# instadeepai/FrameDiPT

Hardware: AMD Instinct MI355X
Metric: residue*diffusion-steps/sec (higher is better)
Workload: dtype fp16

## Files before the change

### framedipt_amd/_lib.py

```python
from __future__ import annotations

import ctypes as C
import os

_HERE = os.path.dirname(os.path.abspath(__file__))
LIB_PATH = os.environ.get("FDIPT_LIB") or os.path.join(_HERE, "lib", "libfdipt_hip.so")

PREC_F32, PREC_BF16, PREC_F16 = 0, 1, 2
PREC_F16X = 3
KF_ET3, KF_GENERIC_PAIR, KF_GENERIC_ATTN, KF_UNFUSED_NODE, KF_UNFOLDED, KF_NO_SPLIT, KF_NO_MERGE, KF_ROWS32, KF_PASS_Z = 1, 2, 4, 8, 16, 32, 64, 128, 256
KF_POINTS_LAUNCH = 512
KF_STREAM_ATTN = 1024
_ERR = {-1: "FDIPT_EINVAL (bad argument)", -2: "FDIPT_ELAUNCH (HIP launch error)",
        -3: "FDIPT_ESIZE (workspace too small or N beyond the compiled tiling: N <= 1024, N <= 2048 with KF_STREAM_ATTN in the fp16 mode; "
            "sample selection: a group of more than 64 samples)"}


class FdiptError(RuntimeError):
    pass


class Dims(C.Structure):
    _fields_ = [(n, C.c_int32) for n in (
        "c_s", "c_z", "c_hidden", "c_skip", "no_heads", "no_qk_points", "no_v_points", "tfmr_heads", "tfmr_layers",
        "num_blocks", "index_embed", "num_bins", "use_aatype", "precision", "kernel_flags")] + [
        (n, C.c_float) for n in ("min_bin", "max_bin", "coordinate_scaling", "r3_min_b", "r3_max_b")]

# ... 153 lines not shown
```

### framedipt_amd/csrc/kernels.hpp

```cpp
#pragma once
#include <hip/hip_runtime.h>
#include <stdint.h>

typedef unsigned short half_t;

struct EdgeTransArgs {
  int B, N;
  const void* z_in;
  void* z_out;
  const float* e;
  const void *w1, *w2, *wf;
  const float *b1, *b2, *bf, *gamma, *beta;
  const float* res_mask;
  float* trace;
  unsigned long long* clock = nullptr;
};

struct EdgeEmbedArgs {
  int B, N, n_rel, rel_off, num_bins;
  const float* pi;
  const float* pj;
  const float* rtab;
  const float* dtab;
  const float* edges;
// ... 212 lines not shown
  float* out = nullptr;
  int ld_out = 0;
  float* out2 = nullptr;
  int ld_out2 = 0, split = 0;
  unsigned short* hid_h16 = nullptr;
  void *img_a = nullptr, *img_b = nullptr;
  int img_B = 0, img_N = 0;
  const float *bb_w = nullptr, *bb_b = nullptr;
  const float* upd_mask = nullptr;
  float *quat = nullptr, *trans = nullptr;
  L2Warm warm = {};
  const void *w3 = nullptr, *w3l = nullptr;
  const float* b3 = nullptr;
  const void *we0 = nullptr, *we0l = nullptr, *we1 = nullptr, *we1l = nullptr;
  const float *be0 = nullptr, *be1 = nullptr;
};
enum { FD_RB_TRANSITION, FD_RB_NODE_EMBED_72, FD_RB_NODE_EMBED_88, FD_RB_TORSION, FD_RB_TRANSITION_BB, FD_RB_ET_ROWS, FD_RB_ET4_ROWS, FD_RB_ET4_IMAGES,
       FD_RB_TRANSITION_BB_SPLIT, FD_RB_NODE_EMBED_72_SPLIT, FD_RB_NODE_EMBED_88_SPLIT, FD_RB_TORSION_SPLIT };
int fd_rowblock(int kind, const RowBlockArgs& a, hipStream_t st);
int fd_transition16(const RowBlockArgs& a, hipStream_t st);
int fd_node_embed16(const RowBlockArgs& a, int k0, hipStream_t st);
int fd_torsion16(const RowBlockArgs& a, hipStream_t st);

struct TfmrTailArgs {
  int M, ld;
  const float *att, *x;
  const void *wo, *w1, *w2;
  const void *wol = nullptr, *w1l = nullptr, *w2l = nullptr, *wpl = nullptr;
  const float *bo, *g1, *be1, *b1, *b2, *g2, *be2;
  float* out;
  const void* wp = nullptr;
  const float *bp = nullptr, *pres = nullptr;
  float* pout = nullptr;
  int ld_pres = 0, ld_pout = 0;
  L2Warm warm;
  int rows16 = 0;
};
int fd_tfmr_tail(const TfmrTailArgs& a, hipStream_t st);
int fd_chain_build_image16(const float* w, int N, int K, int Kpad, int ldw, int lo, void* img, hipStream_t st);

struct ChainArgs {
  int M = 0;
  const float* in = nullptr;
  int ld_in = 0;
  const void* w[3] = {};
  const float* b[3] = {};
  const float* residual = nullptr;
  int ld_res = 0;
  const float *gamma = nullptr, *beta = nullptr;
  unsigned short* out_h16 = nullptr;
  const float* rowmask_pre = nullptr;
  const float* rowmask_post = nullptr;
  float* out = nullptr;
// ... 68 lines not shown
```

### framedipt_amd/csrc/model.hip

```cpp
#include <math.h>
#include <string.h>

#include <vector>

#include "common.hpp"
#include "kernels.hpp"

struct LinW { long w, b; int out, in; };
struct LNW { long g, b; int d; };
#define FD_MAX_BLOCKS 8
#define FD_MAX_TL 4
struct TfLayer { LinW inp, outp, l1, l2; LNW n1, n2; };
struct BlockW {
  long head_w;
  LinW q, kv, qp, kvp, lb, dz, out, rbf;
  LNW ipa_ln;
  LinW skip;
  TfLayer tf[FD_MAX_TL];
  LinW post, t1, t2, t3;
  LNW tln;
  LinW bb;
  LinW et_init, et1, et2, etf;
  LNW et_ln;
};
// ... 565 lines not shown
enum EtRows { ETR_IMAGES, ETR_ROWS, ETR_FOLDED };
struct ForwardPlan {
  int op;
  bool bf, chain, rbk, split;
  NodeForm embed, tail, transition, torsion;
  SkipAt skip;
  OutProj outproj;
  int slices;
  bool feats_fused, ee_bias, et_bias, pz;
  bool stream;
  bool a3, probs_h16;
  bool vpt, proj2, merged, proj_pts, vt_lo, init_fused, feats_h16;
  NodeRows node_rows;
  SeqAttn seq;
  PostAt post;
  bool et_widths;
  EtKind et;
  EtRows et_rows;
  bool torf_fused, bb_fold;
  bool regpair;
  bool ipa_bias_f32, ipa_attn_f32;
  bool x;
  bool refused;
};
static const char kImage = 0;

static ForwardPlan plan_forward(const FdiptDims* d, const Inventory& iv, const DLayout& L, int B, int N, int op) {
  const unsigned f = (unsigned)d->kernel_flags;
  const bool generic_attn = f & FDIPT_KF_GENERIC_ATTN, unfolded = f & FDIPT_KF_UNFOLDED;
  const int cs = d->c_s, cz = d->c_z, H = d->no_heads, C = d->c_hidden, Pq = d->no_qk_points, Pv = d->no_v_points;
// ... 48 lines not shown
  const int th = d->tfmr_heads, hd = iv.d_t / th;
  const bool seq_ok = p.stream ? fd_seq_attention_stream_supported(N, th, hd) : fd_seq_attention_supported(N, th, hd);
  if (p.rbk && !generic_attn && seq_ok && fd_seq_qkv_supported(N, th, iv.d_t)) p.seq = SEQ_FUSED;
  else if (p.bf && !generic_attn && seq_ok) p.seq = SEQ_BF16;
  else if (!p.bf && !generic_attn && fd_seq_attention_f32_supported(N, th, hd, 3 * iv.d_t)) p.seq = SEQ_F32;
  else p.seq = SEQ_GENERIC;
  p.ipa_bias_f32 = !p.bf && H == 8 && cz == 128;
  p.ipa_attn_f32 = !p.bf && !generic_attn;
  p.init_fused = p.proj2 && p.seq == SEQ_FUSED && !unfolded;
  p.feats_h16 = p.a3 && opair_mfma && splitk && (iv.feat_dim & 7) == 0 && !p.split && op == OP_ALL;
  if (!splitk) p.outproj = OUT_GEMM;
  else if (p.split && p.merged && outproj_image(d, iv)) p.outproj = OUT_DEDICATED;
  else p.outproj = p.split ? OUT_SPLITK_SPLIT : p.feats_h16 ? OUT_SPLITK_A16 : OUT_SPLITK;
  p.slices = p.outproj == OUT_DEDICATED ? fd_outproj_split_slices() : p.split ? 3 : 4;
  p.post = p.rbk && !unfolded ? POST_TAIL : p.chain ? POST_CHAIN : POST_GEMM;
  p.torf_fused = (cs & 3) == 0 && !unfolded;
  p.bb_fold = !unfolded;
  p.x = d->precision == FDIPT_PREC_F16X;
  const unsigned x_refused = FDIPT_KF_ET3 | FDIPT_KF_GENERIC_PAIR | FDIPT_KF_GENERIC_ATTN | FDIPT_KF_UNFUSED_NODE | FDIPT_KF_NO_SPLIT |
                             FDIPT_KF_STREAM_ATTN;
  const bool runs_et = op == OP_ALL || op == OP_ET;
  p.refused = p.x && ((f & x_refused) || (runs_et && p.et != ET_ET4) || !p.split || N > 1024);
  return p;
}

enum WarmOf { WARM_QKV, WARM_TAIL, WARM_POST, WARM_TRANSITION, WARM_TRANSITION32, WARM_ET_ROWS, WARM_ET_FOLDED, WARM_TORSION };
struct Fwd {
  const FdiptDims* d;
  const Inventory& iv;
  const DLayout& L;
// ... 17 lines not shown
  int lin32(const LinW& l, const float* A, int lda, float* out, int ldo) const {
    return fd_linear(FDIPT_PREC_F32, R, l.out, l.in, A, lda, P + l.w, l.in, P + l.b, nullptr, 0, nullptr, 0, out, ldo, st);
  }
  int d2d(void* dst, const void* src, size_t bytes) const {
    return hipMemcpyAsync(dst, src, bytes, hipMemcpyDeviceToDevice, st) == hipSuccess ? FDIPT_OK : FDIPT_ELAUNCH;
  }
  int inner(int b, int slot, const float* src, int ld, int cols) const {
    if (!a->trace_inner) return FDIPT_OK;
    float* dst = a->trace_inner + ((size_t)(b * 4 + slot) * R) * iv.d_t;
    return hipMemcpy2DAsync(dst, (size_t)iv.d_t * 4, src, (size_t)ld * 4, (size_t)cols * 4, R, hipMemcpyDeviceToDevice, st) == hipSuccess
               ? FDIPT_OK : FDIPT_ELAUNCH;
  }
  bool first_block(int b) const { return b == 0 || p.op != OP_ALL; }
  bool bias_ready(int b) const { return p.op == OP_ALL && (b == 0 ? p.ee_bias : (p.et == ET_ET3 || p.et == ET_ET4) && p.et_bias); }
  bool fold_et_rows(int b) const { return p.et_rows == ETR_FOLDED && b < d->num_blocks - 1; }
  L2Warm warm_of(int b, WarmOf next, int l = 0) const {
    const DBlock& db = L.blk[b];
    const int cs = d->c_s, dt = iv.d_t;
    const unsigned tb = (unsigned)fd_chain_image_bytes(cs, cs);
    switch (next) {
      case WARM_QKV: {
        const unsigned n = (unsigned)fd_chain_image_bytes(3 * dt, dt);
        return L2Warm{{D + db.ch.inp[l], p.split ? D + db.lo.inp[l] : nullptr, nullptr}, {n, p.split ? n : 0u, 0}};
      }
      case WARM_TAIL: {
        if (p.tail == NF_ROWS16) return L2Warm{{D + db.lo.o16[l][0], D + db.lo.o16[l][1], nullptr}, {db.lo.tail16_run[l], db.lo.tail16_run[l], 0}};
        const unsigned wimg = (unsigned)fd_chain_image_bytes(dt, dt);
        return L2Warm{{D + db.ch.outp[l], D + db.ch.l1[l], D + db.ch.l2[l]}, {wimg, wimg, wimg}};
      }
      case WARM_POST: return L2Warm{{D + db.ch.post, nullptr, nullptr}, {(unsigned)fd_chain_image_bytes(cs, dt), 0, 0}};
// ... 184 lines not shown
    else if (p.outproj == OUT_SPLITK_SPLIT)
      RC(fd_linear_splitk_split(R, cs, feat, p.slices, F(w.feats), feat, wout, feat, bout, res_mask, F(w.ipa_parts), (long)R * cs, cs, st));
    else if (p.outproj == OUT_SPLITK_A16)
      RC(fd_linear_splitk_a16(R, cs, feat, p.slices, (const half_t*)(W + w.feats), feat, WM(k.out), feat, P + k.out.b, res_mask,
                              F(w.ipa_parts), (long)R * cs, cs, st));
    else
      RC(fd_linear_splitk(R, cs, feat, p.slices, F(w.feats), feat, WM(k.out), feat, P + k.out.b, res_mask, F(w.ipa_parts), (long)R * cs, cs, st));
    const bool skip_batched = p.skip != SKIP_PER_BLOCK;
    const L2Warm warm = warm_of(b, WARM_QKV, 0);
    RC(fd_layernorm_parts(R, cs, node, cs, F(w.ipa_parts), cs, p.slices, (long)R * cs, P + k.ipa_ln.g, P + k.ipa_ln.b, nullptr,
                          F(w.tf_in), dt, skip_batched ? F(w.skip_all) + (size_t)b * d->c_skip : nullptr,
                          d->num_blocks * d->c_skip, d->c_skip, p.seq == SEQ_FUSED ? &warm : nullptr, st));
    if (!skip_batched) RC(lin(k.skip, F(w.node0), cs, nullptr, 0, nullptr, 0, F(w.tf_in) + cs, dt));
    return FDIPT_OK;
  }
  int seq_stage(int b, const float** x_out) const {
    const BlockW& k = iv.blk[b];
    const DBlock& db = L.blk[b];
    const int dt = iv.d_t, cs = d->c_s, th = d->tfmr_heads, hd = dt / th;
    const float* x = F(w.tf_in);
    for (int l = 0; l < d->tfmr_layers; ++l) {
      const TfLayer& t = k.tf[l];
      const bool last = l + 1 == d->tfmr_layers;
      if (p.seq == SEQ_FUSED) {
        if (b == 0 && l == 0 && !p.init_fused) RC(fd_seq_images_init(B, N, th, res_mask, W + w.seqimg, SeqInitExtra{}, st, p.stream));
        RC(fd_seq_qkv(B, N, th, x, dt, D + db.ch.inp[l], p.split ? D + db.lo.inp[l] : nullptr, P + t.inp.b, 1.0f / sqrtf((float)hd),
                      W + w.seqimg, st));
        const L2Warm wt = warm_of(b, WARM_TAIL, l);
        RC(fd_seq_attention_run(B, N, th, W + w.seqimg, F(w.att), dt, &wt, st, p.stream));
      } else {
        RC(lin(t.inp, x, dt, nullptr, 0, nullptr, 0, F(w.qkv), 3 * dt));
// ... 18 lines not shown
      const bool r16 = p.tail == NF_ROWS16;
      TfmrTailArgs tt;
      tt.M = R; tt.ld = dt; tt.att = F(w.att); tt.x = x;
      tt.wo = D + (r16 ? db.lo.o16[l][0] : db.ch.outp[l]); tt.w1 = D + (r16 ? db.lo.f16[l][0] : db.ch.l1[l]); tt.w2 = D + (r16 ? db.lo.g16[l][0] : db.ch.l2[l]);
      if (p.split) { tt.wol = D + (r16 ? db.lo.o16[l][1] : db.lo.outp[l]); tt.w1l = D + (r16 ? db.lo.f16[l][1] : db.lo.l1[l]); tt.w2l = D + (r16 ? db.lo.g16[l][1] : db.lo.l2[l]); }
      tt.bo = P + t.outp.b; tt.g1 = P + t.n1.g; tt.be1 = P + t.n1.b; tt.b1 = P + t.l1.b; tt.b2 = P + t.l2.b; tt.g2 = P + t.n2.g;
      tt.be2 = P + t.n2.b; tt.out = x == F(w.x_b) ? F(w.x_a) : F(w.x_b);
      tt.rows16 = r16;
      const bool post_here = last && p.post == POST_TAIL;
      if (post_here) {
        tt.wp = D + (r16 ? db.lo.p16[0] : db.ch.post); tt.wpl = r16 ? D + db.lo.p16[1] : p.split ? D + db.lo.post : nullptr;
        tt.bp = P + k.post.b; tt.pres = F(w.tf_in); tt.ld_pres = dt; tt.pout = F(w.h_a); tt.ld_pout = cs;
      }
      if (!last) tt.warm = p.seq == SEQ_FUSED ? warm_of(b, WARM_QKV, l + 1) : L2Warm{};
      else tt.warm = warm_of(b, post_here ? WARM_TRANSITION : WARM_POST);
      RC(fd_tfmr_tail(tt, st));
      x = tt.out;
    }
    *x_out = x;
    return FDIPT_OK;
  }
  int transition_stage(int b, const float* x) const {
    const BlockW& k = iv.blk[b];
    const DBlock& db = L.blk[b];
    const int cs = d->c_s, dt = iv.d_t;
    if (p.post == POST_CHAIN) {
      ChainArgs c;
      c.M = R; c.in = x; c.ld_in = dt; c.w[0] = D + db.ch.post; c.b[0] = P + k.post.b; c.residual = F(w.tf_in); c.ld_res = dt;
      c.out = F(w.h_a); c.ld_out = cs;
      if (p.rbk) c.warm = warm_of(b, WARM_TRANSITION32);
      RC(fd_chain(FD_CHAIN_POST, c, st));
    } else if (p.post == POST_GEMM) RC(lin(k.post, x, dt, F(w.tf_in), dt, nullptr, 0, F(w.h_a), cs));
    if (p.transition == NF_GEMM) {
      RC(lin(k.t1, F(w.h_a), cs, nullptr, 0, nullptr, 1, F(w.h_b), cs));
      RC(lin(k.t2, F(w.h_b), cs, nullptr, 0, nullptr, 1, F(w.ipa_out), cs));
      RC(lin(k.t3, F(w.ipa_out), cs, F(w.h_a), cs, nullptr, 0, F(w.h_b), cs));
      RC(fd_layernorm(R, cs, F(w.h_b), cs, nullptr, 0, P + k.tln.g, P + k.tln.b, a->res_mask, F(w.node), cs, st));
      RC(lin32(k.bb, F(w.node), cs, F(w.upd), 8));
      RC(inner(b, 3, F(w.upd), 8, 6));
      return fd_compose_q_update(R, F(w.quat), F(w.trans), F(w.upd), 8, F(w.dmask), st);
    }
    const bool r16 = p.transition == NF_ROWS16;
    RowBlockArgs r;
    r.M = R; r.in = F(w.h_a); r.ld_in = cs;
    r.w0 = D + (r16 ? db.lo.tr16[0][0] : db.ch.t1); r.w1 = D + (r16 ? db.lo.tr16[1][0] : db.ch.t2); r.w2 = D + (r16 ? db.lo.tr16[2][0] : db.ch.t3);
    if (p.split) { r.w0l = D + (r16 ? db.lo.tr16[0][1] : db.lo.t1); r.w1l = D + (r16 ? db.lo.tr16[1][1] : db.lo.t2); r.w2l = D + (r16 ? db.lo.tr16[2][1] : db.lo.t3); }
    r.b0 = P + k.t1.b; r.b1 = P + k.t2.b; r.b2 = P + k.t3.b; r.residual = F(w.h_a); r.ld_res = cs; r.gamma = P + k.tln.g; r.beta = P + k.tln.b;
    r.rowmask_post = a->res_mask; r.out = F(w.node); r.ld_out = cs; r.bb_w = P + k.bb.w; r.bb_b = P + k.bb.b;
    r.upd_mask = F(w.dmask); r.quat = F(w.quat); r.trans = F(w.trans);
    if (b < d->num_blocks - 1 && p.et_widths) r.warm = warm_of(b, WARM_ET_ROWS);
    else if (b == d->num_blocks - 1) r.warm = warm_of(b, WARM_TORSION);
    if (fold_et_rows(b)) {
      r.we0 = D + db.lo.ei16[0]; r.we0l = D + db.lo.ei16[1]; r.we1 = D + db.lo.r416[0]; r.we1l = D + db.lo.r416[1];
      r.be0 = P + k.et_init.b; r.be1 = (const float*)(D + db.ch.r4b);
      r.img_a = W + w.a1img; r.img_b = W + w.b1img; r.img_B = B; r.img_N = N;
      r.warm = warm_of(b, WARM_ET_FOLDED);
    }
    if (r16) return fd_transition16(r, st);
    return fd_rowblock(p.split ? FD_RB_TRANSITION_BB_SPLIT : FD_RB_TRANSITION_BB, r, st);
  }
  int edge_transition_stage(int b, const float* node) const {
    const BlockW& k = iv.blk[b];
    const DBlock& db = L.blk[b];
    const int cs = d->c_s, cz = d->c_z;
    RowBlockArgs r;
    r.M = R; r.in = node; r.ld_in = cs; r.w0 = D + db.ch.et_init; r.b0 = P + k.et_init.b;
    if (p.et == ET_ET4 && !fold_et_rows(b)) {
      r.w1 = D + db.ch.r4w; r.b1 = (const float*)(D + db.ch.r4b); r.out = F(w.r4); r.ld_out = 1024;
      r.img_a = W + w.a1img; r.img_b = W + w.b1img; r.img_B = B; r.img_N = N;
      if (p.et_rows == ETR_ROWS) {
        RC(fd_rowblock(FD_RB_ET4_ROWS, r, st));
// ... 34 lines not shown
      t2.clock = a->clock_out;
      if (p.et == ET_ET4) RC(fd_edge_transition4(t2, st, p.x));
      else RC(fd_edge_transition3(t2, st));
    } else {
      EdgeTransArgs ta;
      ta.B = B; ta.N = N; ta.z_in = W + w.z; ta.z_out = W + w.z; ta.e = F(w.e);
      ta.w1 = WM(k.et1); ta.w2 = WM(k.et2); ta.wf = WM(k.etf); ta.b1 = P + k.et1.b; ta.b2 = P + k.et2.b; ta.bf = P + k.etf.b;
      ta.gamma = P + k.et_ln.g; ta.beta = P + k.et_ln.b; ta.res_mask = a->res_mask; ta.trace = tr_ptr; ta.clock = a->clock_out;
      RC(fd_edge_transition(op_precision(d), cz, iv.cb, ta, st));
    }
    if (a->ev_stop && a->ev_stop[b]) hipEventRecord((hipEvent_t)a->ev_stop[b], st);
    return FDIPT_OK;
  }
  int heads_stage(const float* node) const {
    const int cs = d->c_s;
    if (p.torsion == NF_GEMM) {
      RC(lin(iv.tor1, node, cs, nullptr, 0, nullptr, 1, F(w.h_a), cs));
      RC(lin(iv.tor2, F(w.h_a), cs, node, cs, nullptr, 0, F(w.h_b), cs));
    } else {
      const bool r16 = p.torsion == NF_ROWS16;
      RowBlockArgs r;
      r.M = R; r.in = node; r.ld_in = cs; r.w0 = D + (r16 ? L.tor16[0][0] : L.ch_tor1); r.w1 = D + (r16 ? L.tor16[1][0] : L.ch_tor2);
      if (p.split) { r.w0l = D + (r16 ? L.tor16[0][1] : L.lo_tor1); r.w1l = D + (r16 ? L.tor16[1][1] : L.lo_tor2); }
      r.b0 = P + iv.tor1.b; r.b1 = P + iv.tor2.b; r.residual = node; r.ld_res = cs; r.out = F(w.h_b); r.ld_out = cs;
      if (r16) RC(fd_torsion16(r, st));
      else RC(fd_rowblock(p.split ? FD_RB_TORSION_SPLIT : FD_RB_TORSION, r, st));
    }
    if (!p.torf_fused) RC(lin32(iv.torf, F(w.h_b), cs, F(w.psi_un), 8));
    const bool atoms = a->atom37 || a->atom14;
    if (atoms && !a->bb_tables) return FDIPT_EINVAL;
    const bool bb_fold = atoms && p.bb_fold;
// ... 76 lines not shown
    RC(f.ipa_attend(b));
    RC(f.lin(iv.blk[b].out, f.F(w.feats), iv.feat_dim, nullptr, 0, a->res_mask, 0, f.F(w.ipa_out), d->c_s));
    if (!op.out) return FDIPT_EINVAL;
    return f.d2d(op.out, f.F(w.ipa_out), node_bytes);
  }
  const int cs = d->c_s, nsk = d->num_blocks * d->c_skip;
  if (p.skip == SKIP_SPLITK)
    RC(fd_linear_splitk_split(R, nsk, cs, 1, f.F(w.node0), cs, (const float*)(f.D + L.skip_w32), cs, (const float*)(f.D + L.skip_b),
                              nullptr, f.F(w.skip_all), 0, nsk, f.st));
  else if (p.skip == SKIP_GEMM)
    RC(fd_linear(op_precision(d), R, nsk, cs, f.F(w.node0), cs, f.D + L.skip_w, cs, (const float*)(f.D + L.skip_b), nullptr, 0,
                 nullptr, 0, f.F(w.skip_all), nsk, f.st));
  const float* node = f.F(w.node0);
  for (int b = 0; b < d->num_blocks; ++b) {
    const float* x;
    RC(f.ipa_project(b, node));
    RC(f.ipa_attend(b));
    RC(f.ipa_out(b, node));
    RC(f.seq_stage(b, &x));
    RC(f.inner(b, 2, x, iv.d_t, iv.d_t));
    RC(f.transition_stage(b, x));
    node = f.F(w.node);
    if (b < d->num_blocks - 1) RC(f.edge_transition_stage(b, node));
    if (a->trace_node) RC(f.d2d(a->trace_node + (size_t)(b + 1) * R * cs, node, node_bytes));
  }
  return f.heads_stage(node);
}

extern "C" {

int fdipt_score_forward(const FdiptDims* d, const float* P, const void* derived, const void* setup,
                        const FdiptForwardArgs* a, void* workspace, size_t workspace_bytes, fdipt_stream_t stream) {
  return forward_impl(d, P, derived, setup, a, workspace, workspace_bytes, stream, OpSel{});
}

int fdipt_edge_embed_fwd(const FdiptDims* d, const float* P, const void* derived, const void* setup, const FdiptForwardArgs* a,
// ... 56 lines not shown
```

### framedipt_amd/csrc/rowblock.hip

```cpp
#include <type_traits>

#include "common.hpp"
#include "kernels.hpp"

#pragma clang fp contract(off)

#define RB_SROW 144

__host__ __device__ constexpr int rb_max(int a, int b) { return a > b ? a : b; }

template <int K0, int N1, int N2, int NOUT, int FLAGS>
struct RBShape {
  static constexpr int KS0 = (K0 + 15) / 16;
  static constexpr int NL = 1 + (N1 > 0) + (N2 > 0);
  static constexpr int KSMAX = rb_max(KS0, rb_max(N1 / 16, N2 / 16));
  static constexpr int WMAX = rb_max(KS0 * 16, rb_max(N1, N2));
  static constexpr int XROW = WMAX * 2 + 16;
  static constexpr bool LN = (FLAGS & 4) != 0;
  static constexpr int CP = (FLAGS & 64) ? 2 : 1;
  static constexpr int NTO_BLK = NOUT / 32 / CP;
  static constexpr int NTMAX = rb_max(NTO_BLK, rb_max(N1 / 32, N2 / 32));
  static constexpr int NTW = (NTMAX + 3) / 4;
  static constexpr bool BB = (FLAGS & 8) != 0;
  static constexpr bool IMG = (FLAGS & 16) != 0;
// ... 680 lines not shown
        const int r = 8 * it + (lane >> 3);
        const f32x4 o = *(const f32x4*)(stg + r * RB_SROW + 16 * (lane & 7));
        if (row0 + r < a.M) *(f32x4*)(a.out + (long)(row0 + r) * a.ld + 32 * T + 4 * (lane & 7)) = o;
      }
    }
  }
  fd_l2_warm_done(warm_tok);
}

#define RB16_BLOCKS 1
#define T16_KS (TL_D / 32)
#define T16_NT (TL_D / 16)
#define T16_XROW (TL_D * 2 + 32)
#define T16_XLO (16 * T16_XROW)
#define T16_SMEM (4 * T16_XLO + (7 * TL_D + TL_NP) * 4 + 2 * 4 * 16 * 4 + 16)
template <bool POST>
__global__ __launch_bounds__(FD_THREADS, RB16_BLOCKS) void tfmr_tail16_kernel(TfmrTailArgs a) {
  extern __shared__ __attribute__((aligned(16))) char smem[];
  char* xs = smem;
  char* hs = xs + 2 * T16_XLO;
  float* cst = (float*)(hs + 2 * T16_XLO);
  float (*red)[4][16] = (float (*)[4][16])(cst + 7 * TL_D + TL_NP);
  const int tid = threadIdx.x, lane = tid & 63, wave = tid >> 6, lr = lane & 15, fg = lane >> 4;
  const int row0 = blockIdx.x * 16;
  const long grow = row0 + lr < a.M ? row0 + lr : a.M - 1;
  FD_STAMP(0);
  hx8 Wh[2][T16_KS], Wl[2][T16_KS];
  auto w_load = [&](auto BUF, const void* img, const void* img_lo, int T) {
    constexpr int b = decltype(BUF)::value;
#pragma unroll
    for (int s = 0; s < T16_KS; ++s) {
      Wh[b][s] = fd_frag((const char*)img + ((size_t)(T * T16_KS + s) * 64 + lane) * 16);
      Wl[b][s] = fd_frag((const char*)img_lo + ((size_t)(T * T16_KS + s) * 64 + lane) * 16);
// ... 22 lines not shown
      xv[k] = *(const f32x4*)(a.att + (long)gr * a.ld + 4 * c4);
    }
    {
      constexpr int NC = 7 * TL_D + (POST ? TL_NP : 0), NCV = (NC + FD_THREADS - 1) / FD_THREADS;
      float cv[NCV];
#pragma unroll
      for (int k = 0; k < NCV; ++k) {
        const int v = tid + k * FD_THREADS, which = v / TL_D, c = v % TL_D;
        const float* src = which == 0 ? a.bo : which == 1 ? a.g1 : which == 2 ? a.be1 : which == 3 ? a.b1 : which == 4 ? a.b2 : which == 5 ? a.g2 : a.be2;
        cv[k] = v < 7 * TL_D ? src[c] : (POST && v < NC ? a.bp[v - 7 * TL_D] : 0.f);
      }
#pragma unroll
      for (int k = 0; k < NCV; ++k)
        if (tid + k * FD_THREADS < NC) cst[tid + k * FD_THREADS] = cv[k];
    }
#pragma unroll
    for (int k = 0; k < 5; ++k) {
      const int idx = tid + k * FD_THREADS, r = idx / 80, c4 = idx % 80;
      put4(xs, r * T16_XROW + 8 * c4, xv[k][0], xv[k][1], xv[k][2], xv[k][3]);
    }
  }
  f32x4 rv[5];
#pragma unroll
  for (int u = 0; u < 5; ++u) rv[u] = *(const f32x4*)(a.x + grow * a.ld + 16 * (wave + 4 * u) + 4 * fg);
  const unsigned warm_tok = fd_l2_warm(a.warm, blockIdx.x, gridDim.x, tid, FD_THREADS);
  __syncthreads();
  FD_STAMP(1);
  hx8 X[T16_KS];
  const char* xl_base = nullptr;
  auto x_load = [&](const char* buf) {
// ... 113 lines not shown
#pragma unroll
    for (int u = 0; u < 5; ++u)
      put4(hs, lr * T16_XROW + 2 * (16 * (wave + 4 * u) + 4 * fg), acc[u][0], acc[u][1], acc[u][2], acc[u][3]);
    __syncthreads();
    x_load(hs);
#pragma unroll
    for (int u = 0; u < 4; ++u) rvp[u] = *(const f32x4*)(a.pres + grow * a.ld_pres + 16 * (wave + 4 * u) + 4 * fg);
    layer(a.wp, a.wpl, std::integral_constant<int, TL_NP / 16>{});
#pragma unroll
    for (int u = 0; u < 4; ++u) {
      const int f0 = 16 * (wave + 4 * u) + 4 * fg;
      const f32x4 bv = *(const f32x4*)(cst + 7 * TL_D + f0);
      f32x4 o;
#pragma unroll
      for (int i = 0; i < 4; ++i) o[i] = acc[u][i] + bv[i] + rvp[u][i];
      if (row0 + lr < a.M) *(f32x4*)(a.pout + (long)(row0 + lr) * a.ld_pout + f0) = o;
    }
    fd_l2_warm_done(warm_tok);
    return;
  }
#pragma unroll
  for (int u = 0; u < 5; ++u)
    if (row0 + lr < a.M) *(f32x4*)(a.out + (long)(row0 + lr) * a.ld + 16 * (wave + 4 * u) + 4 * fg) = acc[u];
  fd_l2_warm_done(warm_tok);
}

#define TR_D 256
#define TR_KS (TR_D / 32)
#define TR_NT (TR_D / 16)
#define TR_XROW (TR_D * 2 + 32)
#define TR_XLO (16 * TR_XROW)
#define TR_NC (11 * TR_D)
#define TR_SMEM (4 * TR_XLO + TR_NC * 4 + 2 * 4 * 16 * 4 + 4 * 16 * 8 * 4 + 64 + 16)
template <int KS0, int NL, bool LN, bool BB, bool SKIP = false, bool ETR = false>
__global__ __launch_bounds__(FD_THREADS, RB16_BLOCKS) void mlp16_kernel(RowBlockArgs a, int k0) {
  extern __shared__ __attribute__((aligned(16))) char smem[];
  char* xs = smem;
  char* hs = xs + 2 * TR_XLO;
  float* cst = (float*)(hs + 2 * TR_XLO);
  float (*red)[4][16] = (float (*)[4][16])(cst + TR_NC);
  float* red3 = (float*)(red + 2);
  float* pmask = red3 + 4 * 16 * 8;
  const int tid = threadIdx.x, lane = tid & 63, wave = tid >> 6, lr = lane & 15, fg = lane >> 4;
  const int row0 = blockIdx.x * 16;
  const long grow = row0 + lr < a.M ? row0 + lr : a.M - 1;
  hx8 Wh[2][TR_KS], Wl[2][TR_KS];
  auto w_load = [&](auto BUF, auto KSC, const void* img, const void* img_lo, int T) {
    constexpr int b = decltype(BUF)::value, KS = decltype(KSC)::value;
#pragma unroll
    for (int s = 0; s < KS; ++s) {
      Wh[b][s] = fd_frag((const char*)img + ((size_t)(T * KS + s) * 64 + lane) * 16);
      Wl[b][s] = fd_frag((const char*)img_lo + ((size_t)(T * KS + s) * 64 + lane) * 16);
    }
  };
// ... 1 lines not shown
  constexpr std::integral_constant<int, TR_KS> K8C{};
  auto put4 = [&](char* buf, int off, float v0, float v1, float v2, float v3) {
    const float v[4] = {v0, v1, v2, v3};
    hx4 pk, pl;
#pragma unroll
    for (int q = 0; q < 4; ++q) {
      pk[q] = (fd_h)v[q];
      pl[q] = (fd_h)(v[q] - (float)pk[q]);
    }
    *(hx4*)(buf + off) = pk;
    *(hx4*)(buf + TR_XLO + off) = pl;
  };
  constexpr std::integral_constant<int, 0> B0{};
  constexpr std::integral_constant<int, 1> B1{};
  w_load(B0, K0C, a.w0, a.w0l, wave);
  {
    constexpr int C4 = KS0 * 8, NV = (16 * C4 + FD_THREADS - 1) / FD_THREADS;
    f32x4 xv[NV];
#pragma unroll
    for (int k = 0; k < NV; ++k) {
      const int idx = tid + k * FD_THREADS, r = idx / C4, c4 = idx % C4;
      const int gr = row0 + r < a.M ? row0 + r : a.M - 1;
      xv[k] = f32x4{0.f, 0.f, 0.f, 0.f};
      if (idx < 16 * C4 && 4 * c4 < k0) xv[k] = *(const f32x4*)(a.in + (long)gr * a.ld_in + 4 * c4);
    }
    {
      constexpr int NCV = TR_NC / FD_THREADS;
      float cv[NCV];
#pragma unroll
      for (int k = 0; k < NCV; ++k) {
        const int v = tid + k * FD_THREADS, which = v / TR_D, c = v % TR_D;
        cv[k] = which == 0 ? a.b0[c] : which == 1 ? a.b1[c] : which == 2 ? (NL == 3 ? a.b2[c] : 0.f) : which == 3 ? (LN ? a.gamma[c] : 1.f)
                : which == 4 ? (LN ? a.beta[c] : 0.f) : (BB ? a.bb_w[v - 5 * TR_D] : 0.f);
      }
#pragma unroll
      for (int k = 0; k < NCV; ++k) cst[tid + k * FD_THREADS] = cv[k];
    }
    if (tid < 16) pmask[tid] = a.rowmask_post ? a.rowmask_post[row0 + tid < a.M ? row0 + tid : a.M - 1] : 1.f;
#pragma unroll
    for (int k = 0; k < NV; ++k) {
      const int idx = tid + k * FD_THREADS, r = idx / C4, c4 = idx % C4;
      if (idx < 16 * C4) put4(xs, r * TR_XROW + 8 * c4, xv[k][0], xv[k][1], xv[k][2], xv[k][3]);
    }
  }
  f32x4 rv[4];
#pragma unroll
  for (int u = 0; u < 4; ++u) {
    rv[u] = f32x4{0.f, 0.f, 0.f, 0.f};
    if (a.residual) rv[u] = *(const f32x4*)(a.residual + grow * a.ld_res + 16 * (wave + 4 * u) + 4 * fg);
  }
  const unsigned warm_tok = fd_l2_warm(a.warm, blockIdx.x, gridDim.x, tid, FD_THREADS);
  __syncthreads();
  hx8 X[TR_KS];
  const char* xl_base = nullptr;
  auto x_load = [&](auto KSC, const char* buf) {
#pragma unroll
    for (int s = 0; s < decltype(KSC)::value; ++s) X[s] = fd_frag(buf + lr * TR_XROW + (32 * s + 8 * fg) * 2);
    xl_base = buf + TR_XLO + lr * TR_XROW + 16 * fg;
  };
  f32x4 acc[4];
  auto mma = [](hx8 w, hx8 x, f32x4 c) {
    return fd_mfma16(w, x, c);
  };
  auto layer = [&](auto KSC, const void* img, const void* img_lo) {
// ... 65 lines not shown
    mu = (red[0][0][lr] + red[0][1][lr] + red[0][2][lr] + red[0][3][lr]) * (1.0f / TR_D);
#pragma unroll
    for (int u = 0; u < 4; ++u)
#pragma unroll
      for (int i = 0; i < 4; ++i) {
        const float dlt = acc[u][i] - mu;
        s2 += dlt * dlt;
      }
    s2 += __shfl_xor(s2, 16, 64); s2 += __shfl_xor(s2, 32, 64);
    if (fg == 0) red[1][wave][lr] = s2;
    __syncthreads();
    rstd = 1.0f / sqrtf((red[1][0][lr] + red[1][1][lr] + red[1][2][lr] + red[1][3][lr]) * (1.0f / TR_D) + 1e-5f);
  }
  const float pm = pmask[lr];
  float pd[6] = {0.f, 0.f, 0.f, 0.f, 0.f, 0.f};
#pragma unroll
  for (int u = 0; u < 4; ++u) {
    const int f0 = 16 * (wave + 4 * u) + 4 * fg;
    const f32x4 gm = *(const f32x4*)(cst + 3 * TR_D + f0), bt = *(const f32x4*)(cst + 4 * TR_D + f0);
    f32x4 o;
#pragma unroll
    for (int i = 0; i < 4; ++i) o[i] = LN ? ((acc[u][i] - mu) * rstd * gm[i] + bt[i]) * pm : acc[u][i] * pm;
    if (row0 + lr < a.M) *(f32x4*)(a.out + (long)(row0 + lr) * a.ld_out + f0) = o;
    if constexpr (BB) {
#pragma unroll
      for (int k = 0; k < 6; ++k) {
        const f32x4 wv = *(const f32x4*)(cst + 5 * TR_D + k * TR_D + f0);
        pd[k] += (o[0] * wv[0] + o[1] * wv[1]) + (o[2] * wv[2] + o[3] * wv[3]);
      }
    }
  }
  if constexpr (SKIP || ETR) {
    w_load(B0, K8C, SKIP ? a.w3 : a.we0, SKIP ? a.w3l : a.we0l, wave);
#pragma unroll
    for (int u = 0; u < 4; ++u) {
      const int f0 = 16 * (wave + 4 * u) + 4 * fg;
      const f32x4 gm = *(const f32x4*)(cst + 3 * TR_D + f0), bt = *(const f32x4*)(cst + 4 * TR_D + f0);
      put4(hs, lr * TR_XROW + 2 * f0, LN ? ((acc[u][0] - mu) * rstd * gm[0] + bt[0]) * pm : acc[u][0] * pm,
           LN ? ((acc[u][1] - mu) * rstd * gm[1] + bt[1]) * pm : acc[u][1] * pm, LN ? ((acc[u][2] - mu) * rstd * gm[2] + bt[2]) * pm : acc[u][2] * pm,
           LN ? ((acc[u][3] - mu) * rstd * gm[3] + bt[3]) * pm : acc[u][3] * pm);
    }
    __syncthreads();
    x_load(K8C, hs);
    if constexpr (SKIP) {
    layer(K8C, a.w3, a.w3l);
#pragma unroll
    for (int u = 0; u < 4; ++u) {
      const int f0 = 16 * (wave + 4 * u) + 4 * fg;
      const f32x4 bv = *(const f32x4*)(a.b3 + f0);
      f32x4 o;
#pragma unroll
      for (int i = 0; i < 4; ++i) o[i] = acc[u][i] + bv[i];
      if (row0 + lr < a.M) *(f32x4*)(a.out2 + (long)(row0 + lr) * a.ld_out2 + f0) = o;
    }
    }
  }
  if constexpr (ETR) {
    f32x4 ea[2];
    fd_static_for<2>([&](auto U) {
      constexpr int u = decltype(U)::value;
      const int T = wave + 4 * u;
      if constexpr (u == 0) w_load(B1, K8C, a.we0, a.we0l, T + 4);
      f32x4 c = {0.f, 0.f, 0.f, 0.f};
#pragma unroll
      for (int s = 0; s < TR_KS; ++s) c = mma(Wh[u][s], X[s], c);
      {
        hx8 xr[3];
        xr[0] = fd_frag(xl_base);
        xr[1] = fd_frag(xl_base + 64);
// ... 85 lines not shown
    const float dq1 = q0 * upd[0] + q2 * upd[2] - q3 * upd[1];
    const float dq2 = q0 * upd[1] - q1 * upd[2] + q3 * upd[0];
    const float dq3 = q0 * upd[2] + q1 * upd[1] - q2 * upd[0];
    const float R0 = q0 * q0 + q1 * q1 - q2 * q2 - q3 * q3, R1 = 2 * q1 * q2 - 2 * q0 * q3, R2 = 2 * q1 * q3 + 2 * q0 * q2;
    const float R3 = 2 * q1 * q2 + 2 * q0 * q3, R4 = q0 * q0 - q1 * q1 + q2 * q2 - q3 * q3, R5 = 2 * q2 * q3 - 2 * q0 * q1;
    const float R6 = 2 * q1 * q3 - 2 * q0 * q2, R7 = 2 * q2 * q3 + 2 * q0 * q1, R8 = q0 * q0 - q1 * q1 - q2 * q2 + q3 * q3;
    const float d0 = R0 * upd[3] + R1 * upd[4] + R2 * upd[5];
    const float d1 = R3 * upd[3] + R4 * upd[4] + R5 * upd[5];
    const float d2 = R6 * upd[3] + R7 * upd[4] + R8 * upd[5];
    const float n0 = q0 + dq0 * m, n1 = q1 + dq1 * m, n2 = q2 + dq2 * m, n3 = q3 + dq3 * m;
    const float nrm = sqrtf(n0 * n0 + n1 * n1 + n2 * n2 + n3 * n3);
    a.quat[r * 4] = n0 / nrm; a.quat[r * 4 + 1] = n1 / nrm; a.quat[r * 4 + 2] = n2 / nrm; a.quat[r * 4 + 3] = n3 / nrm;
    fd_store3(a.trans + r * 3, a.trans[r * 3] + d0 * m, a.trans[r * 3 + 1] + d1 * m, a.trans[r * 3 + 2] + d2 * m);
  }
  fd_l2_warm_done(warm_tok);
}
template <int KS0, int NL, bool LN, bool BB, bool SKIP = false, bool ETR = false>
static int mlp16_launch(const RowBlockArgs& a, int k0, hipStream_t st) {
  static FdPerDevice attr_dev;
  const int dev_ = fd_device();
  if (!attr_dev.get(dev_)) {
    if (hipFuncSetAttribute((const void*)mlp16_kernel<KS0, NL, LN, BB, SKIP, ETR>, hipFuncAttributeMaxDynamicSharedMemorySize, TR_SMEM) != hipSuccess) return FDIPT_ELAUNCH;
    attr_dev.set(dev_, 1);
  }
  hipLaunchKernelGGL((mlp16_kernel<KS0, NL, LN, BB, SKIP, ETR>), dim3(cdiv(a.M, 16)), dim3(FD_THREADS), TR_SMEM, st, a, k0);
  FD_CHECK_LAUNCH();
  return FDIPT_OK;
}
int fd_transition16(const RowBlockArgs& a, hipStream_t st) {
  if (a.M <= 0 || (a.ld_in & 3) || (a.ld_res & 3) || (a.ld_out & 3) || !a.w0l || !a.w1l || !a.w2l || !a.residual || !a.gamma || !a.beta || !a.bb_w ||
// ... 99 lines not shown
```

### include/fdipt.h

```cpp
#ifndef FDIPT_H
#define FDIPT_H

#include <stddef.h>
#include <stdint.h>

#ifdef __cplusplus
extern "C" {
#endif

#define FDIPT_OK 0
#define FDIPT_EINVAL (-1)
#define FDIPT_ELAUNCH (-2)
#define FDIPT_ESIZE (-3)

#define FDIPT_PREC_F32 0
#define FDIPT_PREC_BF16 1
#define FDIPT_PREC_F16 2
#define FDIPT_PREC_F16X 3

#define FDIPT_KF_ET3 1
#define FDIPT_KF_GENERIC_PAIR 2
#define FDIPT_KF_GENERIC_ATTN 4
#define FDIPT_KF_UNFUSED_NODE 8
#define FDIPT_KF_UNFOLDED 16
#define FDIPT_KF_NO_SPLIT 32
#define FDIPT_KF_NO_MERGE 64
#define FDIPT_KF_ROWS32 128
#define FDIPT_KF_PASS_Z 256
#define FDIPT_KF_POINTS_LAUNCH 512
#define FDIPT_KF_STREAM_ATTN 1024
#define FDIPT_KF_ALL 2047

typedef void* fdipt_stream_t;

typedef struct FdiptDims {
  int32_t c_s;
  int32_t c_z;
  int32_t c_hidden;
  int32_t c_skip;
  int32_t no_heads;
  int32_t no_qk_points;
  int32_t no_v_points;
  int32_t tfmr_heads;
  int32_t tfmr_layers;
  int32_t num_blocks;
  int32_t index_embed;
// ... 267 lines not shown
```

Before: 1.183 million.

## Fuse last transformer tail with node transition and torsion head in one kernel

Adds a fused kernel that runs the last transformer layer's tail (including post projection) and then the node transition MLP/backbone update in the same workgroup. The projected rows stay in registers instead of going out to global memory and being read back. On the final block it also folds the torsion head MLP into the same launch. The aim is to save a kernel launch and a global round trip of the row activations per block. The cost is a larger shared-memory footprint per workgroup, which may lower occupancy, plus more template variants. A flag restores the separate launches.

```diff
diff --git a/framedipt_amd/_lib.py b/framedipt_amd/_lib.py
--- a/framedipt_amd/_lib.py
+++ b/framedipt_amd/_lib.py
@@ -11,6 +11,7 @@
 KF_ET3, KF_GENERIC_PAIR, KF_GENERIC_ATTN, KF_UNFUSED_NODE, KF_UNFOLDED, KF_NO_SPLIT, KF_NO_MERGE, KF_ROWS32, KF_PASS_Z = 1, 2, 4, 8, 16, 32, 64, 128, 256
 KF_POINTS_LAUNCH = 512
 KF_STREAM_ATTN = 1024
+KF_TAIL_LAUNCH = 4096
 _ERR = {-1: "FDIPT_EINVAL (bad argument)", -2: "FDIPT_ELAUNCH (HIP launch error)",
         -3: "FDIPT_ESIZE (workspace too small or N beyond the compiled tiling: N <= 1024, N <= 2048 with KF_STREAM_ATTN in the fp16 mode; "
             "sample selection: a group of more than 64 samples)"}
diff --git a/framedipt_amd/csrc/kernels.hpp b/framedipt_amd/csrc/kernels.hpp
--- a/framedipt_amd/csrc/kernels.hpp
+++ b/framedipt_amd/csrc/kernels.hpp
@@ -250,6 +250,10 @@
   const float* b3 = nullptr;
   const void *we0 = nullptr, *we0l = nullptr, *we1 = nullptr, *we1l = nullptr;
   const float *be0 = nullptr, *be1 = nullptr;
+  const void *wt0 = nullptr, *wt0l = nullptr, *wt1 = nullptr, *wt1l = nullptr;
+  const float *bt0 = nullptr, *bt1 = nullptr;
+  float* out_t = nullptr;
+  int ld_out_t = 0;
 };
 enum { FD_RB_TRANSITION, FD_RB_NODE_EMBED_72, FD_RB_NODE_EMBED_88, FD_RB_TORSION, FD_RB_TRANSITION_BB, FD_RB_ET_ROWS, FD_RB_ET4_ROWS, FD_RB_ET4_IMAGES,
        FD_RB_TRANSITION_BB_SPLIT, FD_RB_NODE_EMBED_72_SPLIT, FD_RB_NODE_EMBED_88_SPLIT, FD_RB_TORSION_SPLIT };
@@ -273,6 +277,7 @@
   int rows16 = 0;
 };
 int fd_tfmr_tail(const TfmrTailArgs& a, hipStream_t st);
+int fd_tail_transition16(const TfmrTailArgs& t, const RowBlockArgs& a, hipStream_t st);
 int fd_chain_build_image16(const float* w, int N, int K, int Kpad, int ldw, int lo, void* img, hipStream_t st);
 
 struct ChainArgs {
diff --git a/framedipt_amd/csrc/model.hip b/framedipt_amd/csrc/model.hip
--- a/framedipt_amd/csrc/model.hip
+++ b/framedipt_amd/csrc/model.hip
@@ -603,6 +603,7 @@
   NodeRows node_rows;
   SeqAttn seq;
   PostAt post;
+  bool tail_fold;
   bool et_widths;
   EtKind et;
   EtRows et_rows;
@@ -681,6 +682,8 @@
   else p.outproj = p.split ? OUT_SPLITK_SPLIT : p.feats_h16 ? OUT_SPLITK_A16 : OUT_SPLITK;
   p.slices = p.outproj == OUT_DEDICATED ? fd_outproj_split_slices() : p.split ? 3 : 4;
   p.post = p.rbk && !unfolded ? POST_TAIL : p.chain ? POST_CHAIN : POST_GEMM;
+  p.tail_fold = p.tail == NF_ROWS16 && p.transition == NF_ROWS16 && p.post == POST_TAIL && d->tfmr_layers > 0 && op == OP_ALL && !unfolded &&
+                !(f & FDIPT_KF_TAIL_LAUNCH);
   p.torf_fused = (cs & 3) == 0 && !unfolded;
   p.bb_fold = !unfolded;
   p.x = d->precision == FDIPT_PREC_F16X;
@@ -728,6 +731,7 @@
   bool first_block(int b) const { return b == 0 || p.op != OP_ALL; }
   bool bias_ready(int b) const { return p.op == OP_ALL && (b == 0 ? p.ee_bias : (p.et == ET_ET3 || p.et == ET_ET4) && p.et_bias); }
   bool fold_et_rows(int b) const { return p.et_rows == ETR_FOLDED && b < d->num_blocks - 1; }
+  bool fold_torsion() const { return p.tail_fold && p.torsion == NF_ROWS16; }
   L2Warm warm_of(int b, WarmOf next, int l = 0) const {
     const DBlock& db = L.blk[b];
     const int cs = d->c_s, dt = iv.d_t;
@@ -942,7 +946,7 @@
     if (!skip_batched) RC(lin(k.skip, F(w.node0), cs, nullptr, 0, nullptr, 0, F(w.tf_in) + cs, dt));
     return FDIPT_OK;
   }
-  int seq_stage(int b, const float** x_out) const {
+  int seq_stage(int b, const float** x_out, TfmrTailArgs* held) const {
     const BlockW& k = iv.blk[b];
     const DBlock& db = L.blk[b];
     const int dt = iv.d_t, cs = d->c_s, th = d->tfmr_heads, hd = dt / th;
@@ -991,13 +995,14 @@
       }
       if (!last) tt.warm = p.seq == SEQ_FUSED ? warm_of(b, WARM_QKV, l + 1) : L2Warm{};
       else tt.warm = warm_of(b, post_here ? WARM_TRANSITION : WARM_POST);
-      RC(fd_tfmr_tail(tt, st));
+      if (last && p.tail_fold) *held = tt;
+      else RC(fd_tfmr_tail(tt, st));
       x = tt.out;
     }
     *x_out = x;
     return FDIPT_OK;
   }
-  int transition_stage(int b, const float* x) const {
+  int transition_stage(int b, const float* x, const TfmrTailArgs& held) const {
     const BlockW& k = iv.blk[b];
     const DBlock& db = L.blk[b];
     const int cs = d->c_s, dt = iv.d_t;
@@ -1019,10 +1024,11 @@
     }
     const bool r16 = p.transition == NF_ROWS16;
     RowBlockArgs r;
-    r.M = R; r.in = F(w.h_a); r.ld_in = cs;
+    r.M = R;
+    if (!p.tail_fold) { r.in = F(w.h_a); r.ld_in = cs; r.residual = F(w.h_a); r.ld_res = cs; }
     r.w0 = D + (r16 ? db.lo.tr16[0][0] : db.ch.t1); r.w1 = D + (r16 ? db.lo.tr16[1][0] : db.ch.t2); r.w2 = D + (r16 ? db.lo.tr16[2][0] : db.ch.t3);
     if (p.split) { r.w0l = D + (r16 ? db.lo.tr16[0][1] : db.lo.t1); r.w1l = D + (r16 ? db.lo.tr16[1][1] : db.lo.t2); r.w2l = D + (r16 ? db.lo.tr16[2][1] : db.lo.t3); }
-    r.b0 = P + k.t1.b; r.b1 = P + k.t2.b; r.b2 = P + k.t3.b; r.residual = F(w.h_a); r.ld_res = cs; r.gamma = P + k.tln.g; r.beta = P + k.tln.b;
+    r.b0 = P + k.t1.b; r.b1 = P + k.t2.b; r.b2 = P + k.t3.b; r.gamma = P + k.tln.g; r.beta = P + k.tln.b;
     r.rowmask_post = a->res_mask; r.out = F(w.node); r.ld_out = cs; r.bb_w = P + k.bb.w; r.bb_b = P + k.bb.b;
     r.upd_mask = F(w.dmask); r.quat = F(w.quat); r.trans = F(w.trans);
     if (b < d->num_blocks - 1 && p.et_widths) r.warm = warm_of(b, WARM_ET_ROWS);
@@ -1032,6 +1038,13 @@
       r.be0 = P + k.et_init.b; r.be1 = (const float*)(D + db.ch.r4b);
       r.img_a = W + w.a1img; r.img_b = W + w.b1img; r.img_B = B; r.img_N = N;
       r.warm = warm_of(b, WARM_ET_FOLDED);
+    }
+    if (p.tail_fold) {
+      if (b == d->num_blocks - 1 && fold_torsion()) {
+        r.wt0 = D + L.tor16[0][0]; r.wt0l = D + L.tor16[0][1]; r.wt1 = D + L.tor16[1][0]; r.wt1l = D + L.tor16[1][1];
+        r.bt0 = P + iv.tor1.b; r.bt1 = P + iv.tor2.b; r.out_t = F(w.h_b); r.ld_out_t = cs;
+      }
+      return fd_tail_transition16(held, r, st);
     }
     if (r16) return fd_transition16(r, st);
     return fd_rowblock(p.split ? FD_RB_TRANSITION_BB_SPLIT : FD_RB_TRANSITION_BB, r, st);
@@ -1096,7 +1109,8 @@
   }
   int heads_stage(const float* node) const {
     const int cs = d->c_s;
-    if (p.torsion == NF_GEMM) {
+    if (fold_torsion()) {
+    } else if (p.torsion == NF_GEMM) {
       RC(lin(iv.tor1, node, cs, nullptr, 0, nullptr, 1, F(w.h_a), cs));
       RC(lin(iv.tor2, F(w.h_a), cs, node, cs, nullptr, 0, F(w.h_b), cs));
     } else {
@@ -1203,12 +1217,13 @@
   const float* node = f.F(w.node0);
   for (int b = 0; b < d->num_blocks; ++b) {
     const float* x;
+    TfmrTailArgs held = {};
     RC(f.ipa_project(b, node));
     RC(f.ipa_attend(b));
     RC(f.ipa_out(b, node));
-    RC(f.seq_stage(b, &x));
+    RC(f.seq_stage(b, &x, &held));
     RC(f.inner(b, 2, x, iv.d_t, iv.d_t));
-    RC(f.transition_stage(b, x));
+    RC(f.transition_stage(b, x, held));
     node = f.F(w.node);
     if (b < d->num_blocks - 1) RC(f.edge_transition_stage(b, node));
     if (a->trace_node) RC(f.d2d(a->trace_node + (size_t)(b + 1) * R * cs, node, node_bytes));
diff --git a/framedipt_amd/csrc/rowblock.hip b/framedipt_amd/csrc/rowblock.hip
--- a/framedipt_amd/csrc/rowblock.hip
+++ b/framedipt_amd/csrc/rowblock.hip
@@ -718,9 +718,8 @@
 #define T16_XROW (TL_D * 2 + 32)
 #define T16_XLO (16 * T16_XROW)
 #define T16_SMEM (4 * T16_XLO + (7 * TL_D + TL_NP) * 4 + 2 * 4 * 16 * 4 + 16)
-template <bool POST>
-__global__ __launch_bounds__(FD_THREADS, RB16_BLOCKS) void tfmr_tail16_kernel(TfmrTailArgs a) {
-  extern __shared__ __attribute__((aligned(16))) char smem[];
+template <bool POST, bool FUSED, class StageMore>
+__device__ __forceinline__ void tfmr_tail16_body(const TfmrTailArgs& a, char* smem, f32x4 (&po)[4], StageMore&& stage_more) {
   char* xs = smem;
   char* hs = xs + 2 * T16_XLO;
   float* cst = (float*)(hs + 2 * T16_XLO);
@@ -773,6 +772,7 @@
       for (int k = 0; k < NCV; ++k)
         if (tid + k * FD_THREADS < NC) cst[tid + k * FD_THREADS] = cv[k];
     }
+    stage_more();
 #pragma unroll
     for (int k = 0; k < 5; ++k) {
       const int idx = tid + k * FD_THREADS, r = idx / 80, c4 = idx % 80;
@@ -916,7 +916,8 @@
       f32x4 o;
 #pragma unroll
       for (int i = 0; i < 4; ++i) o[i] = acc[u][i] + bv[i] + rvp[u][i];
-      if (row0 + lr < a.M) *(f32x4*)(a.pout + (long)(row0 + lr) * a.ld_pout + f0) = o;
+      if constexpr (FUSED) po[u] = o;
+      else if (row0 + lr < a.M) *(f32x4*)(a.pout + (long)(row0 + lr) * a.ld_pout + f0) = o;
     }
     fd_l2_warm_done(warm_tok);
     return;
@@ -925,6 +926,12 @@
   for (int u = 0; u < 5; ++u)
     if (row0 + lr < a.M) *(f32x4*)(a.out + (long)(row0 + lr) * a.ld + 16 * (wave + 4 * u) + 4 * fg) = acc[u];
   fd_l2_warm_done(warm_tok);
+}
+template <bool POST>
+__global__ __launch_bounds__(FD_THREADS, RB16_BLOCKS) void tfmr_tail16_kernel(TfmrTailArgs a) {
+  extern __shared__ __attribute__((aligned(16))) char smem[];
+  f32x4 po[4];
+  tfmr_tail16_body<POST, false>(a, smem, po, [] {});
 }
 
 #define TR_D 256
@@ -934,12 +941,26 @@
 #define TR_XLO (16 * TR_XROW)
 #define TR_NC (11 * TR_D)
 #define TR_SMEM (4 * TR_XLO + TR_NC * 4 + 2 * 4 * 16 * 4 + 4 * 16 * 8 * 4 + 64 + 16)
-template <int KS0, int NL, bool LN, bool BB, bool SKIP = false, bool ETR = false>
-__global__ __launch_bounds__(FD_THREADS, RB16_BLOCKS) void mlp16_kernel(RowBlockArgs a, int k0) {
-  extern __shared__ __attribute__((aligned(16))) char smem[];
-  char* xs = smem;
+template <int NL, bool LN, bool BB>
+__device__ __forceinline__ void mlp16_consts(const RowBlockArgs& a, float* cst) {
+  const int tid = threadIdx.x, row0 = blockIdx.x * 16;
+  float* pmask = cst + TR_NC + 2 * 4 * 16 + 4 * 16 * 8;
+  constexpr int NCV = TR_NC / FD_THREADS;
+  float cv[NCV];
+#pragma unroll
+  for (int k = 0; k < NCV; ++k) {
+    const int v = tid + k * FD_THREADS, which = v / TR_D, c = v % TR_D;
+    cv[k] = which == 0 ? a.b0[c] : which == 1 ? a.b1[c] : which == 2 ? (NL == 3 ? a.b2[c] : 0.f) : which == 3 ? (LN ? a.gamma[c] : 1.f)
+            : which == 4 ? (LN ? a.beta[c] : 0.f) : (BB ? a.bb_w[v - 5 * TR_D] : 0.f);
+  }
+#pragma unroll
+  for (int k = 0; k < NCV; ++k) cst[tid + k * FD_THREADS] = cv[k];
+  if (tid < 16) pmask[tid] = a.rowmask_post ? a.rowmask_post[row0 + tid < a.M ? row0 + tid : a.M - 1] : 1.f;
+}
+template <int KS0, int NL, bool LN, bool BB, bool SKIP, bool ETR, bool FUSED, bool TOR>
+__device__ __forceinline__ void mlp16_body(const RowBlockArgs& a, int k0, char* xs, float* cst, const f32x4 (&pin)[4]) {
+  static_assert(!TOR || (FUSED && !ETR && !SKIP), "the torsion stages ride on the fused launch's plain form");
   char* hs = xs + 2 * TR_XLO;
-  float* cst = (float*)(hs + 2 * TR_XLO);
   float (*red)[4][16] = (float (*)[4][16])(cst + TR_NC);
   float* red3 = (float*)(red + 2);
   float* pmask = red3 + 4 * 16 * 8;
@@ -971,7 +992,15 @@
   constexpr std::integral_constant<int, 0> B0{};
   constexpr std::integral_constant<int, 1> B1{};
   w_load(B0, K0C, a.w0, a.w0l, wave);
-  {
+  f32x4 rv[4];
+  if constexpr (FUSED) {
+    static_assert(KS0 == TR_KS, "the rows in registers are 256 wide");
+#pragma unroll
+    for (int u = 0; u < 4; ++u) {
+      put4(xs, lr * TR_XROW + 2 * (16 * (wave + 4 * u) + 4 * fg), pin[u][0], pin[u][1], pin[u][2], pin[u][3]);
+      rv[u] = pin[u];
+    }
+  } else {
     constexpr int C4 = KS0 * 8, NV = (16 * C4 + FD_THREADS - 1) / FD_THREADS;
     f32x4 xv[NV];
 #pragma unroll
@@ -981,30 +1010,17 @@
       xv[k] = f32x4{0.f, 0.f, 0.f, 0.f};
       if (idx < 16 * C4 && 4 * c4 < k0) xv[k] = *(const f32x4*)(a.in + (long)gr * a.ld_in + 4 * c4);
     }
-    {
-      constexpr int NCV = TR_NC / FD_THREADS;
-      float cv[NCV];
-#pragma unroll
-      for (int k = 0; k < NCV; ++k) {
-        const int v = tid + k * FD_THREADS, which = v / TR_D, c = v % TR_D;
-        cv[k] = which == 0 ? a.b0[c] : which == 1 ? a.b1[c] : which == 2 ? (NL == 3 ? a.b2[c] : 0.f) : which == 3 ? (LN ? a.gamma[c] : 1.f)
-                : which == 4 ? (LN ? a.beta[c] : 0.f) : (BB ? a.bb_w[v - 5 * TR_D] : 0.f);
-      }
-#pragma unroll
-      for (int k = 0; k < NCV; ++k) cst[tid + k * FD_THREADS] = cv[k];
-    }
-    if (tid < 16) pmask[tid] = a.rowmask_post ? a.rowmask_post[row0 + tid < a.M ? row0 + tid : a.M - 1] : 1.f;
+    mlp16_consts<NL, LN, BB>(a, cst);
 #pragma unroll
     for (int k = 0; k < NV; ++k) {
       const int idx = tid + k * FD_THREADS, r = idx / C4, c4 = idx % C4;
       if (idx < 16 * C4) put4(xs, r * TR_XROW + 8 * c4, xv[k][0], xv[k][1], xv[k][2], xv[k][3]);
     }
-  }
-  f32x4 rv[4];
-#pragma unroll
-  for (int u = 0; u < 4; ++u) {
-    rv[u] = f32x4{0.f, 0.f, 0.f, 0.f};
-    if (a.residual) rv[u] = *(const f32x4*)(a.residual + grow * a.ld_res + 16 * (wave + 4 * u) + 4 * fg);
+#pragma unroll
+    for (int u = 0; u < 4; ++u) {
+      rv[u] = f32x4{0.f, 0.f, 0.f, 0.f};
+      if (a.residual) rv[u] = *(const f32x4*)(a.residual + grow * a.ld_res + 16 * (wave + 4 * u) + 4 * fg);
+    }
   }
   const unsigned warm_tok = fd_l2_warm(a.warm, blockIdx.x, gridDim.x, tid, FD_THREADS);
   __syncthreads();
@@ -1100,6 +1116,7 @@
   }
   const float pm = pmask[lr];
   float pd[6] = {0.f, 0.f, 0.f, 0.f, 0.f, 0.f};
+  f32x4 nr[TOR ? 4 : 1];
 #pragma unroll
   for (int u = 0; u < 4; ++u) {
     const int f0 = 16 * (wave + 4 * u) + 4 * fg;
@@ -1108,6 +1125,7 @@
 #pragma unroll
     for (int i = 0; i < 4; ++i) o[i] = LN ? ((acc[u][i] - mu) * rstd * gm[i] + bt[i]) * pm : acc[u][i] * pm;
     if (row0 + lr < a.M) *(f32x4*)(a.out + (long)(row0 + lr) * a.ld_out + f0) = o;
+    if constexpr (TOR) nr[u] = o;
     if constexpr (BB) {
 #pragma unroll
       for (int k = 0; k < 6; ++k) {
@@ -1116,13 +1134,14 @@
       }
     }
   }
-  if constexpr (SKIP || ETR) {
-    w_load(B0, K8C, SKIP ? a.w3 : a.we0, SKIP ? a.w3l : a.we0l, wave);
+  if constexpr (SKIP || ETR || TOR) {
+    w_load(B0, K8C, SKIP ? a.w3 : TOR ? a.wt0 : a.we0, SKIP ? a.w3l : TOR ? a.wt0l : a.we0l, wave);
 #pragma unroll
     for (int u = 0; u < 4; ++u) {
       const int f0 = 16 * (wave + 4 * u) + 4 * fg;
       const f32x4 gm = *(const f32x4*)(cst + 3 * TR_D + f0), bt = *(const f32x4*)(cst + 4 * TR_D + f0);
-      put4(hs, lr * TR_XROW + 2 * f0, LN ? ((acc[u][0] - mu) * rstd * gm[0] + bt[0]) * pm : acc[u][0] * pm,
+      if constexpr (TOR) put4(hs, lr * TR_XROW + 2 * f0, nr[u][0], nr[u][1], nr[u][2], nr[u][3]);
+      else put4(hs, lr * TR_XROW + 2 * f0, LN ? ((acc[u][0] - mu) * rstd * gm[0] + bt[0]) * pm : acc[u][0] * pm,
            LN ? ((acc[u][1] - mu) * rstd * gm[1] + bt[1]) * pm : acc[u][1] * pm, LN ? ((acc[u][2] - mu) * rstd * gm[2] + bt[2]) * pm : acc[u][2] * pm,
            LN ? ((acc[u][3] - mu) * rstd * gm[3] + bt[3]) * pm : acc[u][3] * pm);
     }
@@ -1139,6 +1158,23 @@
       for (int i = 0; i < 4; ++i) o[i] = acc[u][i] + bv[i];
       if (row0 + lr < a.M) *(f32x4*)(a.out2 + (long)(row0 + lr) * a.ld_out2 + f0) = o;
     }
+    }
+    if constexpr (TOR) {
+      layer(K8C, a.wt0, a.wt0l);
+      w_load(B0, K8C, a.wt1, a.wt1l, wave);
+      relu_to(xs, a.bt0);
+      __syncthreads();
+      x_load(K8C, xs);
+      layer(K8C, a.wt1, a.wt1l);
+#pragma unroll
+      for (int u = 0; u < 4; ++u) {
+        const int f0 = 16 * (wave + 4 * u) + 4 * fg;
+        const f32x4 bv = *(const f32x4*)(a.bt1 + f0);
+        f32x4 o;
+#pragma unroll
+        for (int i = 0; i < 4; ++i) o[i] = acc[u][i] + bv[i] + nr[u][i];
+        if (row0 + lr < a.M) *(f32x4*)(a.out_t + (long)(row0 + lr) * a.ld_out_t + f0) = o;
+      }
     }
   }
   if constexpr (ETR) {
@@ -1254,6 +1290,43 @@
     fd_store3(a.trans + r * 3, a.trans[r * 3] + d0 * m, a.trans[r * 3 + 1] + d1 * m, a.trans[r * 3 + 2] + d2 * m);
   }
   fd_l2_warm_done(warm_tok);
+}
+template <int KS0, int NL, bool LN, bool BB, bool SKIP = false, bool ETR = false>
+__global__ __launch_bounds__(FD_THREADS, RB16_BLOCKS) void mlp16_kernel(RowBlockArgs a, int k0) {
+  extern __shared__ __attribute__((aligned(16))) char smem[];
+  const f32x4 none[4] = {};
+  mlp16_body<KS0, NL, LN, BB, SKIP, ETR, false, false>(a, k0, smem, (float*)(smem + 4 * TR_XLO), none);
+}
+#define TT16_SMEM (T16_SMEM + TR_SMEM - 4 * TR_XLO)
+template <bool ETR, bool TOR>
+__global__ __launch_bounds__(FD_THREADS, RB16_BLOCKS) void tail_transition16_kernel(TfmrTailArgs t, RowBlockArgs a) {
+  extern __shared__ __attribute__((aligned(16))) char smem[];
+  float* cst = (float*)(smem + T16_SMEM);
+  f32x4 h[4];
+  tfmr_tail16_body<true, true>(t, smem, h, [&] { mlp16_consts<3, true, true>(a, cst); });
+  mlp16_body<8, 3, true, true, false, ETR, true, TOR>(a, TR_D, smem, cst, h);
+}
+int fd_tail_transition16(const TfmrTailArgs& t, const RowBlockArgs& a, hipStream_t st) {
+  if (t.M <= 0 || t.M != a.M || (t.ld & 3) || !t.wol || !t.w1l || !t.w2l || !t.wp || !t.wpl || !t.bp || !t.pres || (t.ld_pres & 3)) return FDIPT_EINVAL;
+  if ((a.ld_out & 3) || !a.w0l || !a.w1l || !a.w2l || !a.gamma || !a.beta || !a.bb_w || !a.bb_b || !a.quat || !a.trans) return FDIPT_EINVAL;
+  const bool etr = a.we0 != nullptr, tor = a.wt0 != nullptr;
+  if (etr && (tor || !a.we0l || !a.we1 || !a.we1l || !a.be0 || !a.be1 || !a.img_a || !a.img_b || (a.img_N & 3) || a.M != a.img_B * a.img_N)) return FDIPT_EINVAL;
+  if (tor && (!a.wt0l || !a.wt1 || !a.wt1l || !a.bt0 || !a.bt1 || !a.out_t || (a.ld_out_t & 3))) return FDIPT_EINVAL;
+  static FdPerDevice attr_dev;
+  const int dev_ = fd_device();
+  if (!attr_dev.get(dev_)) {
+    if (hipFuncSetAttribute((const void*)tail_transition16_kernel<false, false>, hipFuncAttributeMaxDynamicSharedMemorySize, TT16_SMEM) != hipSuccess ||
+        hipFuncSetAttribute((const void*)tail_transition16_kernel<true, false>, hipFuncAttributeMaxDynamicSharedMemorySize, TT16_SMEM) != hipSuccess ||
+        hipFuncSetAttribute((const void*)tail_transition16_kernel<false, true>, hipFuncAttributeMaxDynamicSharedMemorySize, TT16_SMEM) != hipSuccess)
+      return FDIPT_ELAUNCH;
+    attr_dev.set(dev_, 1);
+  }
+  const dim3 grid(cdiv(a.M, 16)), block(FD_THREADS);
+  if (etr) hipLaunchKernelGGL((tail_transition16_kernel<true, false>), grid, block, TT16_SMEM, st, t, a);
+  else if (tor) hipLaunchKernelGGL((tail_transition16_kernel<false, true>), grid, block, TT16_SMEM, st, t, a);
+  else hipLaunchKernelGGL((tail_transition16_kernel<false, false>), grid, block, TT16_SMEM, st, t, a);
+  FD_CHECK_LAUNCH();
+  return FDIPT_OK;
 }
 template <int KS0, int NL, bool LN, bool BB, bool SKIP = false, bool ETR = false>
 static int mlp16_launch(const RowBlockArgs& a, int k0, hipStream_t st) {
diff --git a/include/fdipt.h b/include/fdipt.h
--- a/include/fdipt.h
+++ b/include/fdipt.h
@@ -29,7 +29,8 @@
 #define FDIPT_KF_PASS_Z 256
 #define FDIPT_KF_POINTS_LAUNCH 512
 #define FDIPT_KF_STREAM_ATTN 1024
-#define FDIPT_KF_ALL 2047
+#define FDIPT_KF_TAIL_LAUNCH 4096
+#define FDIPT_KF_ALL 6143
 
 typedef void* fdipt_stream_t;
 
```

Result: no change. 1.188 million (median of 6 runs) (+0.5%).
